# FibonacciDude/ContrastiveProsthetics

Measured on AMD Instinct MI355X. Metric: sEMG windows/sec contrastive step, 12-ch Ninapro, 1/2/4/8 MI355X, higher is better.
Workload: dtype bf16; 1 GPU; synthetic 12-ch sEMG, 41-class one-hot, batch 4096 groups/GPU (167936 windows/GPU/step), stock BN (--no_adabn), dp_emg=0.0635, d_e=16, random-init weights; global_batch_groups=4096, parallelism=dp1, loss=reference per-group loss, tile_schedule=static

## Files before the change

### contrastiveprosthetics_amd/csrc/conv_kernels.cuh

```cuda
#pragma once
#include <type_traits>
#include "common.cuh"
#include "gemm_tn.cuh"

#define CONV_WPB 16
#define CONV_ROWS (CONV_WPB * 12)
#define CONV_IMG_ROWS (CONV_WPB * 14)

struct ConvArgs {
    const float* x;
    const float* w1;
    const float* b1;
    const float* stats1;
    const void* wc;
    const float* bias2;
    const void* gin;
    const int* gin_exp;
    const float* coef;
    void* out;
    uint8_t* out8;
    const int* out_exp;
    uint32_t* out_amax;
    float* partials;
    int64_t n_windows;
// ... 449 lines not shown
    if constexpr (G8) gd = f8_exp2i(-*a.gin_exp);
    auto prefetch = [&](int64_t strip) {
        const int64_t win0 = strip * CONV_WG_WPB;
#pragma unroll
        for (int q = 0; q < NIT; ++q) {
            const int ir = rr + q * RPP;
            const int nl = ir / 14, wp = ir % 14;
            const int64_t win = win0 + nl;
            const bool ok = strip < nstrips && ir < CONV_WG_IMG && wp >= 1 && wp <= 12 && win < a.n_windows;
            const int64_t winc = ok ? win : 0;
            const int wpos = ok ? wp - 1 : 0;
            xg[q] = *(const GV*)((const unsigned char*)a.gin + ((winc * 12 + wpos) * 64 + cc * EPC) * (int64_t)sizeof(GV) / EPC);
            if constexpr (BN2) xr2[q] = *(const uint4*)((const T*)a.r2 + (winc * 12 + wpos) * 64 + cc * EPC);
            const float* xw = a.x + winc * 12;
            xr[q][0] = xw[wpos > 0 ? wpos - 1 : 0];
            xr[q][1] = xw[wpos];
            xr[q][2] = xw[wpos < 11 ? wpos + 1 : 11];
        }
    };
    prefetch(blockIdx.x);
    for (int64_t strip = blockIdx.x; strip < nstrips; strip += gridDim.x) {
        const int64_t win0 = strip * CONV_WG_WPB;
        {
#pragma unroll
            for (int q = 0; q < NIT; ++q) {
                const int ir = rr + q * RPP;
                const int nl = ir / 14, wp = ir % 14;
                const bool ok = ir < CONV_WG_IMG && wp >= 1 && wp <= 12 && win0 + nl < a.n_windows;
                const int wpos = ok ? wp - 1 : 0;
                float t[EPC];
                conv1_chunk_vals<T>(wpos > 0 ? xr[q][0] : 0.f, xr[q][1], wpos < 11 ? xr[q][2] : 0.f, wt, bs, t);
                if (a.stats1 != nullptr) {
#pragma unroll
                    for (int e = 0; e < EPC; ++e) t[e] = fmaf(t[e], sc[e], sh[e]);
                }
                uint4 yv = D::pack(t);
                uint4 xv;
                if constexpr (G8) xv = f8_chunk5_to_bf16(xg[q], gd);
                else xv = xg[q];
                if constexpr (BN2) {
                    float gv[EPC], rv[EPC];
                    D::unpack(xv, gv);
                    D::unpack(xr2[q], rv);
#pragma unroll
                    for (int e = 0; e < EPC; ++e) gv[e] = rv[e] > 0.f ? fmaf(c2a[e], gv[e], fmaf(c2b[e], rv[e], c2z[e])) : 0.f;
                    xv = D::pack(gv);
                    if (ok) {
                        *(uint4*)((T*)const_cast<void*>(a.gin) + ((win0 + nl) * 12 + wpos) * 64 + cc * EPC) = xv;
                        D::unpack(xv, gv);
#pragma unroll
                        for (int e = 0; e < EPC; ++e) {
                            cs_all[e] += gv[e];
                            cs_first[e] += wpos == 0 ? gv[e] : 0.f;
                            cs_last[e] += wpos == 11 ? gv[e] : 0.f;
                        }
                    }
                }
                if (!ok) { xv = make_uint4(0, 0, 0, 0); yv = make_uint4(0, 0, 0, 0); }
                if (ir < CONV_WG_IMG) {
                    *(uint4*)(Xi + (ir + 1) * PITCH + cc * 16) = xv;
                    *(uint4*)(Yi + (ir + 1) * PITCH + cc * 16) = yv;
                }
            }
        }
        __syncthreads();
        prefetch(strip + gridDim.x);
#pragma unroll
        for (int k0 = 0; k0 < CONV_WG_IMG; k0 += KSTEP) {
            uint4 fy;
            if constexpr (sizeof(T) == 2) fy = tn_frag_bf16<PITCH>(Yi, k0 + 1, it * 32, lane);
            else fy = tn_frag_f32<PITCH>(Yi, k0 + 1, it * 32, lane);
#pragma unroll
            for (int tap = 0; tap < 3; ++tap) {
                uint4 fx;
                if constexpr (sizeof(T) == 2) fx = tn_frag_bf16<PITCH>(Xi, k0 + 2 - tap, ot * 32, lane);
                else fx = tn_frag_f32<PITCH>(Xi, k0 + 2 - tap, ot * 32, lane);
                mma_chunk<T>(fx, fy, acc[tap]);
            }
        }
        __syncthreads();
    }
    float* slab = a.partials + (int64_t)blockIdx.x * 64 * 192;
    const int r = lane & 31, h = lane >> 5;
#pragma unroll
    for (int tap = 0; tap < 3; ++tap) {
        const int q = tap * 64 + it * 32 + r;
#pragma unroll
        for (int g = 0; g < 16; ++g) {
            const int p = ot * 32 + (g & 3) + 8 * (g >> 2) + 4 * h;
            slab[p * 192 + q] = acc[tap][g];
        }
    }
    if constexpr (BN2) {
        float* red = (float*)smem;
        static_assert(2 * ROWS * PITCH >= 3 * RPP * 64 * 4, "the column-sum reduction reuses the image region");
#pragma unroll
        for (int e = 0; e < EPC; ++e) {
            red[(0 * RPP + rr) * 64 + cc * EPC + e] = cs_all[e];
            red[(1 * RPP + rr) * 64 + cc * EPC + e] = cs_first[e];
            red[(2 * RPP + rr) * 64 + cc * EPC + e] = cs_last[e];
        }
        __syncthreads();
        if (tid < 192) {
            const int which = tid >> 6, c = tid & 63;
            float s = 0.f;
            for (int q = 0; q < RPP; ++q) s += red[(which * RPP + q) * 64 + c];
            a.gcols3[((int64_t)blockIdx.x * 3 + which) * 64 + c] = s;
        }
    }
}

template <typename T, bool G8 = false, bool ROWS = false>
__global__ __launch_bounds__(256, 2) void conv2_dgrad_conv1_kernel(ConvArgs a) {
    static_assert(!G8 || sizeof(T) == 2, "e5m2 gradients are expanded into a bf16 image");
    using GV = std::conditional_t<G8, uint2, uint4>;
    using D = DT<T>;
    using G = ConvGeo<T>;
    constexpr int EPC = G::EPC, CPR = G::CPR, ROWB = G::ROWB, RPP = G::RPP, WPITCH = G::WPITCH;
    constexpr int KSTEP = D::KSTEP, KS_PER_TAP = 64 / KSTEP, NKS = 3 * KS_PER_TAP;
    constexpr int IMG_BYTES = CONV_IMG_ROWS * ROWB, W_BYTES = 64 * WPITCH;
    __shared__ __attribute__((aligned(16))) unsigned char smem[IMG_BYTES + W_BYTES];
    __shared__ __attribute__((aligned(16))) float xpad[2][CONV_WPB * 16];
    static_assert(IMG_BYTES >= 4 * 8 * 32 * 4, "the end-of-kernel reduction reuses the image region");
    unsigned char* img = smem;
    unsigned char* Wl = smem + IMG_BYTES;
    float* red = (float*)smem;

    const int tid = threadIdx.x, lane = tid & 63, wave = tid >> 6;
    const int r = lane & 31, h = lane >> 5;
    const int cc = tid % CPR, rr = tid / CPR;
    const int ft = wave & 1, st0 = 3 * (wave >> 1);
    const int64_t nstrips = (a.n_windows + CONV_WPB - 1) / CONV_WPB;
    const int64_t total_rows = a.n_windows * 12;

    for (int i = tid; i < 64 * (192 / EPC); i += 256) {
        const int row = i / (192 / EPC), ch = i % (192 / EPC);
        *(uint4*)(Wl + row * WPITCH + ch * 16) = *(const uint4*)((const T*)a.wc + row * 192 + ch * EPC);
    }
    for (int i = tid; i < 2 * CONV_WPB * 16; i += 256) (&xpad[0][0])[i] = 0.f;
    const int ch1 = ft * 32 + r;
    const float w0 = a.w1[ch1 * 9 + 3], w1 = a.w1[ch1 * 9 + 4], w2 = a.w1[ch1 * 9 + 5], b1 = a.b1[ch1];
    float ca, cb, cz;
    if constexpr (ROWS) {
        __shared__ float ca_s[64], cb_s[64], cz_s[64];
        conv_bn_bwd_coef(a.rows1, a.rows1_nr, 1, a.stats1, (double)a.n_windows * 12, ca_s, cb_s, cz_s, (double (*)[4][64])smem, blockIdx.x == 0,
                         a.dgamma1, a.dbeta1);
        ca = ca_s[ch1]; cb = cb_s[ch1]; cz = cz_s[ch1];
        __syncthreads();
    } else {
        ca = a.coef[ch1]; cb = a.coef[64 + ch1]; cz = a.coef[128 + ch1];
    }
    float d0 = 0.f, d1 = 0.f, d2 = 0.f, d3 = 0.f;

    auto load_x = [&](int64_t strip) {
        const int64_t i = strip * (CONV_WPB * 12) + tid;
        return (tid < CONV_WPB * 12 && strip < nstrips && i < total_rows) ? a.x[i] : 0.f;
    };
    const int xslot = (tid / 12) * 16 + 1 + tid % 12;
    constexpr int NITG = CONV_IMG_ROWS / RPP;
    GV pg[NITG];
    float gd = 1.f;
    if constexpr (G8) gd = f8_exp2i(-*a.gin_exp);
    auto prefetch_g = [&](int64_t strip) {
#pragma unroll
        for (int it = 0; it < NITG; ++it) {
            const int ir = rr + it * RPP;
            const int nl = ir / 14, wp = ir % 14;
            const int64_t win = strip * CONV_WPB + nl;
            const bool ok = strip < nstrips && wp >= 1 && wp <= 12 && win < a.n_windows;
            pg[it] = *(const GV*)((const unsigned char*)a.gin + (((ok ? win : 0) * 12 + (ok ? wp - 1 : 0)) * 64 + cc * EPC) * (int64_t)sizeof(GV) / EPC);
            if (!ok) pg[it] = GV{};
        }
    };
    __syncthreads();
    if (tid < CONV_WPB * 12) xpad[0][xslot] = load_x(blockIdx.x);
    prefetch_g(blockIdx.x);
    int xb = 0;
    int ir0[3];
#pragma unroll
    for (int j = 0; j < 3; ++j) {
        const int ml = (st0 + j) * 32 + r;
        ir0[j] = (ml / 12) * 14 + (ml % 12);
    }
    for (int64_t strip = blockIdx.x; strip < nstrips; strip += gridDim.x) {
        const int64_t win0 = strip * CONV_WPB;
        const float x_next = load_x(strip + gridDim.x);
#pragma unroll
        for (int it = 0; it < NITG; ++it) {
            if constexpr (G8) *(uint4*)(img + G::img_off(rr + it * RPP, cc)) = f8_chunk5_to_bf16(pg[it], gd);
            else *(uint4*)(img + G::img_off(rr + it * RPP, cc)) = pg[it];
        }
        __syncthreads();
        prefetch_g(strip + gridDim.x);
        f32x16 acc[3];
#pragma unroll
        for (int j = 0; j < 3; ++j)
#pragma unroll
            for (int g = 0; g < 16; ++g) acc[j][g] = 0.f;
#pragma unroll
        for (int ks = 0; ks < NKS; ++ks) {
            const int tap = ks / KS_PER_TAP, chunk = (ks % KS_PER_TAP) * 2 + h;
            const uint4 fw = *(const uint4*)(Wl + (ft * 32 + r) * WPITCH + ks * 32 + h * 16);
#pragma unroll
            for (int j = 0; j < 3; ++j) {
                const uint4 fs = *(const uint4*)(img + G::img_off(ir0[j] + tap, chunk));
                mma_chunk<T>(fs, fw, acc[j]);
            }
        }
        if (tid < CONV_WPB * 12) xpad[xb ^ 1][xslot] = x_next;
        __syncthreads();
        const float* xs = xpad[xb];
#pragma unroll
        for (int j = 0; j < 3; ++j) {
#pragma unroll
            for (int q = 0; q < 4; ++q) {
                const int mb = (st0 + j) * 32 + 8 * q + 4 * h;
                const int nl = mb / 12, p0 = mb % 12;
                const bool valid = win0 + nl < a.n_windows;
                const float4 xa = *(const float4*)(xs + nl * 16 + p0);
                const float2 xc = *(const float2*)(xs + nl * 16 + p0 + 4);
                const float X[6] = {xa.x, xa.y, xa.z, xa.w, xc.x, xc.y};
#pragma unroll
                for (int e = 0; e < 4; e += 2) {
                    float y0 = fmaf(w2, X[e + 2], fmaf(w1, X[e + 1], fmaf(w0, X[e], b1)));
                    float y1 = fmaf(w2, X[e + 3], fmaf(w1, X[e + 2], fmaf(w0, X[e + 1], b1)));
                    float r0, r1;
                    if constexpr (sizeof(T) == 2) {
                        const uint32_t pk = cvt_pk_bf16<true>(y0, y1);
                        r0 = __uint_as_float(pk << 16);
                        r1 = __uint_as_float(pk & 0xffff0000u);
                    } else {
                        r0 = fmaxf(y0, 0.f);
                        r1 = fmaxf(y1, 0.f);
                    }
                    const float t0 = fmaf(ca, acc[j][4 * q + e], fmaf(cb, r0, cz));
                    const float t1 = fmaf(ca, acc[j][4 * q + e + 1], fmaf(cb, r1, cz));
                    const float g0 = (r0 > 0.f && valid) ? t0 : 0.f;
                    const float g1 = (r1 > 0.f && valid) ? t1 : 0.f;
                    d0 = fmaf(g0, X[e], d0);     d1 = fmaf(g0, X[e + 1], d1); d2 = fmaf(g0, X[e + 2], d2); d3 += g0;
                    d0 = fmaf(g1, X[e + 1], d0); d1 = fmaf(g1, X[e + 2], d1); d2 = fmaf(g1, X[e + 3], d2); d3 += g1;
                }
                __builtin_amdgcn_sched_barrier(0);
            }
        }
        xb ^= 1;
    }
    __syncthreads();
    red[(0 * 8 + wave * 2 + h) * 32 + r] = d0;
    red[(1 * 8 + wave * 2 + h) * 32 + r] = d1;
    red[(2 * 8 + wave * 2 + h) * 32 + r] = d2;
    red[(3 * 8 + wave * 2 + h) * 32 + r] = d3;
    __syncthreads();
    {
        const int k = tid >> 6, c = tid & 63, f = c >> 5, cl = c & 31;
        float s = 0.f;
#pragma unroll
        for (int wq = 0; wq < 2; ++wq)
#pragma unroll
            for (int hh = 0; hh < 2; ++hh) s += red[(k * 8 + (f + 2 * wq) * 2 + hh) * 32 + cl];
        a.partials[((int64_t)blockIdx.x * 4 + k) * 64 + c] = s;
    }
}
```

### contrastiveprosthetics_amd/csrc/gemm_nt.cuh

```cuda
#pragma once
#include "common.cuh"

enum { ALOAD_PLAIN = 0, ALOAD_CONV = 1,
       ALOAD_BNDROP = 2,
       ALOAD_F8 = 3,
       ALOAD_BNDROP_F8 = 4 };
enum { EPI_FWD = 0, EPI_DGRAD = 1, EPI_PLAIN_F32 = 2,
       EPI_DGRAD_BN = 3,
       EPI_DGRAD_ST = 4 };

struct GemmNTArgs {
    const void* A;
    const void* W;
    void* C;
    const float* bias;
    const void* R;
    float* partials;
    const float* coef;
    int coef_mod;
    const float* a_scale;
    const float* a_shift;
    const int* a_exp;
    int64_t M;
    int lda, ldc, ldr;
    int K, F;
    int relu;
    int f_valid;
    int pad0;
    uint32_t dp_thresh, dp_key;
    const uint32_t* dp_salt;
    float dp_inv_keep;
    int* sched;
};

template <typename T, int BM, int BN, int ALOAD, int EPI>
__global__ __launch_bounds__(256) void gemm_nt_kernel(GemmNTArgs a) {
    using D = DT<T>;
    constexpr int EPC = D::EPC;
    constexpr int BK = D::BK;
    constexpr int WAVES_F = (BN >= 128) ? 2 : 1;
    constexpr int WAVES_S = 4 / WAVES_F;
    constexpr int WS_T = BM / (WAVES_S * 32);
    constexpr int WF_T = BN / (WAVES_F * 32);
    constexpr int A_BYTES = BM * 128, W_BYTES = BN * 128;
    constexpr int C_PITCH = BN * (int)sizeof(T) + 16;
    constexpr int STAGE_BYTES = 2 * (A_BYTES + W_BYTES);
    constexpr int C_BYTES = (EPI == EPI_PLAIN_F32) ? 0 : BM * C_PITCH;
    constexpr int RED_BYTES = (EPI == EPI_PLAIN_F32) ? 0 : 2 * 256 * EPC * 4;
    constexpr int LDS_BYTES = (STAGE_BYTES > C_BYTES + RED_BYTES) ? STAGE_BYTES : (C_BYTES + RED_BYTES);
    static_assert(LDS_BYTES <= 160 * 1024, "LDS");
    __shared__ __attribute__((aligned(16))) unsigned char smem[LDS_BYTES];

    const int tid = threadIdx.x, lane = tid & 63, wave = tid >> 6;
    const int r = lane & 31, h = lane >> 5;
    const int tiles_f = a.F / BN;
    const int tile_f = blockIdx.x % tiles_f;
    const int64_t tile_m = blockIdx.x / tiles_f;
    const int64_t m0 = tile_m * BM;
    const int f0 = tile_f * BN;
    const int ws = wave / WAVES_F, wf = wave % WAVES_F;

    const T* __restrict__ Ag = (const T*)a.A;
    const T* __restrict__ Wg = (const T*)a.W;

    constexpr int A_IT = BM / 32, W_IT = BN / 32;
    uint4 areg[A_IT], wreg[W_IT];
    const int sc = tid & 7, sr = tid >> 3;
    float a_deq = 1.f;
    if constexpr (ALOAD == ALOAD_F8 || ALOAD == ALOAD_BNDROP_F8) a_deq = f8_exp2i(-*a.a_exp);

    auto load_tiles = [&](int kt) {
        const int k0 = kt * BK;
#pragma unroll
        for (int i = 0; i < W_IT; ++i) {
            const int row = sr + 32 * i;
            wreg[i] = *(const uint4*)(Wg + (int64_t)(f0 + row) * a.K + k0 + sc * EPC);
        }
#pragma unroll
        for (int i = 0; i < A_IT; ++i) {
            const int64_t m = m0 + sr + 32 * i;
            if constexpr (ALOAD == ALOAD_PLAIN || ALOAD == ALOAD_BNDROP || ALOAD == ALOAD_F8 || ALOAD == ALOAD_BNDROP_F8) {
                const int64_t mc = m < a.M ? m : a.M - 1;
                uint4 v;
                if constexpr (ALOAD == ALOAD_F8 || ALOAD == ALOAD_BNDROP_F8) {
                    static_assert(sizeof(T) == 2 || (ALOAD != ALOAD_F8 && ALOAD != ALOAD_BNDROP_F8), "e4m3 operands feed the bf16 kernels");
                    v = f8_chunk_to_bf16(*(const uint2*)((const uint8_t*)a.A + mc * a.lda + k0 + sc * 8), a_deq);
                } else {
                    v = *(const uint4*)(Ag + mc * a.lda + k0 + sc * EPC);
                }
                if constexpr (ALOAD == ALOAD_BNDROP || ALOAD == ALOAD_BNDROP_F8)
                    v = bn_drop_chunk<T>(v, a.a_scale, a.a_shift, k0 + sc * EPC, a.dp_salt ? (a.dp_key ^ *a.dp_salt) : a.dp_key, (uint32_t)mc,
                                         (uint32_t)a.K, a.dp_thresh, a.dp_inv_keep);
                if (m >= a.M) v = make_uint4(0, 0, 0, 0);
                areg[i] = v;
            } else {
                const int tap = k0 >> 6, ch0 = (k0 & 63) + sc * EPC;
                const int w = (int)(m % 12) + tap - 1;
                const bool ok = (m < a.M) && (w >= 0) && (w < 12);
                const int64_t ms = ok ? (m + tap - 1) : 0;
                uint4 v = *(const uint4*)(Ag + ms * a.lda + ch0);
                if (a.a_scale != nullptr) {
                    float x[EPC];
                    D::unpack(v, x);
#pragma unroll
                    for (int e = 0; e < EPC; ++e) x[e] = fmaf(x[e], a.a_scale[ch0 + e], a.a_shift[ch0 + e]);
                    v = D::pack(x);
                }
                if (!ok) v = make_uint4(0, 0, 0, 0);
                areg[i] = v;
            }
        }
    };
    auto store_tiles = [&](int buf) {
        unsigned char* As = smem + buf * (A_BYTES + W_BYTES);
        unsigned char* Ws = As + A_BYTES;
#pragma unroll
        for (int i = 0; i < A_IT; ++i) *(uint4*)(As + lds_tile_off(sr + 32 * i, sc)) = areg[i];
#pragma unroll
        for (int i = 0; i < W_IT; ++i) *(uint4*)(Ws + lds_tile_off(sr + 32 * i, sc)) = wreg[i];
    };

    f32x16 acc[WF_T][WS_T];
#pragma unroll
    for (int i = 0; i < WF_T; ++i)
#pragma unroll
        for (int j = 0; j < WS_T; ++j)
#pragma unroll
            for (int g = 0; g < 16; ++g) acc[i][j][g] = 0.f;

    const int nk = a.K / BK;
    load_tiles(0);
    store_tiles(0);
    __syncthreads();
    for (int kt = 0; kt < nk; ++kt) {
        if (kt + 1 < nk) load_tiles(kt + 1);
        const unsigned char* As = smem + (kt & 1) * (A_BYTES + W_BYTES);
        const unsigned char* Ws = As + A_BYTES;
#pragma unroll
        for (int ks = 0; ks < 4; ++ks) {
            uint4 fw[WF_T], fs[WS_T];
#pragma unroll
            for (int i = 0; i < WF_T; ++i)
                fw[i] = *(const uint4*)(Ws + lds_tile_off((wf * WF_T + i) * 32 + r, 2 * ks + h));
#pragma unroll
            for (int j = 0; j < WS_T; ++j)
                fs[j] = *(const uint4*)(As + lds_tile_off((ws * WS_T + j) * 32 + r, 2 * ks + h));
#pragma unroll
            for (int i = 0; i < WF_T; ++i)
#pragma unroll
                for (int j = 0; j < WS_T; ++j) mma_chunk<T>(fw[i], fs[j], acc[i][j]);
        }
        if (kt + 1 < nk) store_tiles((kt + 1) & 1);
        __syncthreads();
    }

    if constexpr (EPI == EPI_PLAIN_F32) {
        float* Cg = (float*)a.C;
#pragma unroll
        for (int i = 0; i < WF_T; ++i)
#pragma unroll
            for (int j = 0; j < WS_T; ++j) {
                const int64_t m = m0 + (ws * WS_T + j) * 32 + r;
#pragma unroll
                for (int q = 0; q < 4; ++q) {
                    const int f = f0 + (wf * WF_T + i) * 32 + 8 * q + 4 * h;
                    if (m < a.M && f < a.f_valid) {
                        float4 v = make_float4(acc[i][j][4 * q], acc[i][j][4 * q + 1], acc[i][j][4 * q + 2], acc[i][j][4 * q + 3]);
                        if (a.bias != nullptr) { v.x += a.bias[f]; v.y += a.bias[f + 1]; v.z += a.bias[f + 2]; v.w += a.bias[f + 3]; }
                        *(float4*)(Cg + m * a.ldc + f) = v;
                    }
                }
            }
        return;
    } else {
        unsigned char* Cs = smem;
        float* red = (float*)(smem + C_BYTES);
#pragma unroll
        for (int i = 0; i < WF_T; ++i)
#pragma unroll
            for (int j = 0; j < WS_T; ++j) {
                const int srow = (ws * WS_T + j) * 32 + r;
#pragma unroll
                for (int q = 0; q < 4; ++q) {
                    const int fl = (wf * WF_T + i) * 32 + 8 * q + 4 * h;
                    float v[4];
#pragma unroll
                    for (int e = 0; e < 4; ++e) {
                        float x = acc[i][j][4 * q + e];
                        if constexpr (EPI == EPI_FWD) {
                            x += a.bias[f0 + fl + e];
                            if (a.relu) x = fmaxf(x, 0.f);
                        }
                        v[e] = x;
                    }
                    unsigned char* dst = Cs + srow * C_PITCH + fl * (int)sizeof(T);
                    if constexpr (sizeof(T) == 2) {
                        *(uint2*)dst = make_uint2(pack2bf(v[0], v[1]), pack2bf(v[2], v[3]));
                    } else {
                        *(float4*)dst = make_float4(v[0], v[1], v[2], v[3]);
                    }
                }
            }
        __syncthreads();
        constexpr int CPR = BN / EPC;
        constexpr int RPP = 256 / CPR;
        const int cc = tid % CPR, rr = tid / CPR;
        float s1[EPC], s2[EPC];
#pragma unroll
        for (int e = 0; e < EPC; ++e) s1[e] = s2[e] = 0.f;
        T* Cg = (T*)a.C;
        const T* Rg = (const T*)a.R;
#pragma unroll 2
        for (int p = 0; p < BM / RPP; ++p) {
            const int row = rr + p * RPP;
            const int64_t m = m0 + row;
            if (m < a.M) {
                uint4 c = *(const uint4*)(Cs + row * C_PITCH + cc * 16);
                float v[EPC];
                D::unpack(c, v);
                const int f = f0 + cc * EPC;
                if constexpr (EPI == EPI_FWD) {
#pragma unroll
                    for (int e = 0; e < EPC; ++e) { s1[e] += v[e]; s2[e] = fmaf(v[e], v[e], s2[e]); }
                } else {
                    float rv[EPC];
                    uint4 rc = make_uint4(0, 0, 0, 0);
                    if (a.R != nullptr) rc = *(const uint4*)(Rg + m * a.ldr + f);
                    D::unpack(rc, rv);
                    if (a.dp_thresh != 0) {
#pragma unroll
                        for (int e = 0; e < EPC; e += 2) {
                            const uint32_t pr = dropout_pair(a.dp_salt ? (a.dp_key ^ *a.dp_salt) : a.dp_key, (uint32_t)m, (uint32_t)a.ldc, (uint32_t)(f + e));
                            v[e] *= dropout_scale(pr, 0, a.dp_thresh, a.dp_inv_keep);
                            v[e + 1] *= dropout_scale(pr, 1, a.dp_thresh, a.dp_inv_keep);
                        }
                        c = D::pack(v);
                    }
#pragma unroll
                    for (int e = 0; e < EPC; ++e) {
                        const float g = D::round(v[e]);
                        s1[e] += g;
                        s2[e] = fmaf(g, rv[e], s2[e]);
                    }
                }
                *(uint4*)(Cg + m * a.ldc + f) = c;
            }
        }
        if (EPI == EPI_DGRAD && a.R == nullptr) return;
#pragma unroll
        for (int e = 0; e < EPC; ++e) {
            red[(0 * RPP + rr) * BN + cc * EPC + e] = s1[e];
            red[(1 * RPP + rr) * BN + cc * EPC + e] = s2[e];
        }
        __syncthreads();
        if (tid < 2 * BN) {
            const int which = tid / BN, col = tid % BN;
            float s = 0.f;
#pragma unroll
            for (int q = 0; q < RPP; ++q) s += red[(which * RPP + q) * BN + col];
            a.partials[(tile_m * 2 + which) * a.F + f0 + col] = s;
        }
    }
}

template <typename T, int BM, int BN, int ALOAD, int EPI>
static inline hipError_t launch_gemm_nt(const GemmNTArgs& a, hipStream_t st) {
    const int64_t tiles_m = (a.M + BM - 1) / BM;
    const int64_t blocks = tiles_m * (a.F / BN);
    hipLaunchKernelGGL((gemm_nt_kernel<T, BM, BN, ALOAD, EPI>), dim3((unsigned)blocks), dim3(256), 0, st, a);
    return hipGetLastError();
}
```

### contrastiveprosthetics_amd/csrc/gemm_tn.cuh

```cuda
#pragma once
#include "common.cuh"

enum { YLOAD_PLAIN = 0, YLOAD_CONV = 1,
       YLOAD_BNDROP = 2,
       YLOAD_F8 = 3,
       YLOAD_BNDROP_F8 = 4 };

struct GemmTNArgs {
    const void* X;
    const void* Y;
    float* slabs;
    const float* y_scale;
    const float* y_shift;
    const int* y_exp;
    int64_t M;
    int64_t rows_per_split;
    int ldx, ldy, P, Q;
    uint32_t dp_thresh, dp_key;
    const uint32_t* dp_salt;
    float dp_inv_keep;
};

template <typename T, int COLS> struct TNPitch {
    static constexpr int value = (sizeof(T) == 2) ? COLS * 2 + 64 : COLS * 4 + 16;
// ... 39 lines not shown
    const int tp = blockIdx.x / tiles_q, tq = blockIdx.x % tiles_q;
    const int p0 = tp * BP, q0 = tq * BQ;
    const int64_t mb = (int64_t)blockIdx.y * a.rows_per_split;
    int64_t me = mb + a.rows_per_split;
    if (me > a.M) me = a.M;
    const int nsteps = (int)((me - mb + 31) / 32);

    const T* __restrict__ Xg = (const T*)a.X;
    const T* __restrict__ Yg = (const T*)a.Y;
    uint4 xreg[X_IT], yreg[Y_IT];
    float y_deq = 1.f;
    if constexpr (YLOAD == YLOAD_F8 || YLOAD == YLOAD_BNDROP_F8) y_deq = f8_exp2i(-*a.y_exp);

    auto load_tiles = [&](int step) {
        const int64_t ms = mb + (int64_t)step * 32;
#pragma unroll
        for (int i = 0; i < X_IT; ++i) {
            const int idx = tid + 256 * i;
            const int row = idx / XCPR, ch = idx % XCPR;
            const int64_t m = ms + row;
            uint4 v = make_uint4(0, 0, 0, 0);
            if (row < 32 && m < me) v = *(const uint4*)(Xg + m * a.ldx + p0 + ch * EPC);
            xreg[i] = v;
        }
#pragma unroll
        for (int i = 0; i < Y_IT; ++i) {
            const int idx = tid + 256 * i;
            const int row = idx / YCPR, ch = idx % YCPR;
            const int64_t m = ms + row;
            uint4 v = make_uint4(0, 0, 0, 0);
            if constexpr (YLOAD == YLOAD_PLAIN) {
                if (row < 32 && m < me) v = *(const uint4*)(Yg + m * a.ldy + q0 + ch * EPC);
            } else if constexpr (YLOAD == YLOAD_F8 || YLOAD == YLOAD_BNDROP_F8) {
                static_assert(sizeof(T) == 2 || (YLOAD != YLOAD_F8 && YLOAD != YLOAD_BNDROP_F8), "e4m3 operands feed the bf16 kernels");
                if (row < 32 && m < me) {
                    v = f8_chunk_to_bf16(*(const uint2*)((const uint8_t*)a.Y + m * a.ldy + q0 + ch * 8), y_deq);
                    if constexpr (YLOAD == YLOAD_BNDROP_F8)
                        v = bn_drop_chunk<T>(v, a.y_scale, a.y_shift, q0 + ch * EPC, a.dp_salt ? (a.dp_key ^ *a.dp_salt) : a.dp_key, (uint32_t)m,
                                             (uint32_t)a.Q, a.dp_thresh, a.dp_inv_keep);
                }
            } else if constexpr (YLOAD == YLOAD_BNDROP) {
                if (row < 32 && m < me)
                    v = bn_drop_chunk<T>(*(const uint4*)(Yg + m * a.ldy + q0 + ch * EPC), a.y_scale, a.y_shift, q0 + ch * EPC,
                                         a.dp_salt ? (a.dp_key ^ *a.dp_salt) : a.dp_key, (uint32_t)m, (uint32_t)a.Q, a.dp_thresh, a.dp_inv_keep);
            } else {
                const int tap = tq;
                const int w = (int)(m % 12) + tap - 1;
                if (row < 32 && m < me && w >= 0 && w < 12) {
                    v = *(const uint4*)(Yg + (m + tap - 1) * a.ldy + ch * EPC);
                    if (a.y_scale != nullptr) {
                        float x[EPC];
                        D::unpack(v, x);
#pragma unroll
                        for (int e = 0; e < EPC; ++e) x[e] = fmaf(x[e], a.y_scale[ch * EPC + e], a.y_shift[ch * EPC + e]);
                        v = D::pack(x);
                    }
                }
            }
            yreg[i] = v;
        }
    };
    auto store_tiles = [&](int buf) {
        unsigned char* Xs = smem + buf * (XB + YB);
        unsigned char* Ys = Xs + XB;
#pragma unroll
        for (int i = 0; i < X_IT; ++i) {
            const int idx = tid + 256 * i;
            const int row = idx / XCPR, ch = idx % XCPR;
            if (row < 32) *(uint4*)(Xs + row * PX + ch * 16) = xreg[i];
        }
#pragma unroll
        for (int i = 0; i < Y_IT; ++i) {
            const int idx = tid + 256 * i;
            const int row = idx / YCPR, ch = idx % YCPR;
            if (row < 32) *(uint4*)(Ys + row * PY + ch * 16) = yreg[i];
        }
    };

    f32x16 acc[WP_T][WQ_T];
#pragma unroll
    for (int i = 0; i < WP_T; ++i)
#pragma unroll
        for (int j = 0; j < WQ_T; ++j)
#pragma unroll
            for (int g = 0; g < 16; ++g) acc[i][j][g] = 0.f;

    if (nsteps > 0) {
        load_tiles(0);
        store_tiles(0);
    }
    __syncthreads();
    for (int step = 0; step < nsteps; ++step) {
        if (step + 1 < nsteps) load_tiles(step + 1);
        const unsigned char* Xs = smem + (step & 1) * (XB + YB);
        const unsigned char* Ys = Xs + XB;
#pragma unroll
        for (int ks = 0; ks < 32 / KSTEP; ++ks) {
            uint4 fx[WP_T], fy[WQ_T];
#pragma unroll
            for (int i = 0; i < WP_T; ++i) {
                const int c0 = (wp * WP_T + i) * 32;
                if constexpr (sizeof(T) == 2) fx[i] = tn_frag_bf16<PX>(Xs, ks * KSTEP, c0, lane);
                else fx[i] = tn_frag_f32<PX>(Xs, ks * KSTEP, c0, lane);
            }
#pragma unroll
            for (int j = 0; j < WQ_T; ++j) {
                const int c0 = (wq * WQ_T + j) * 32;
                if constexpr (sizeof(T) == 2) fy[j] = tn_frag_bf16<PY>(Ys, ks * KSTEP, c0, lane);
                else fy[j] = tn_frag_f32<PY>(Ys, ks * KSTEP, c0, lane);
            }
#pragma unroll
            for (int i = 0; i < WP_T; ++i)
#pragma unroll
                for (int j = 0; j < WQ_T; ++j) mma_chunk<T>(fx[i], fy[j], acc[i][j]);
        }
        if (step + 1 < nsteps) store_tiles((step + 1) & 1);
        __syncthreads();
    }

    float* slab = a.slabs + (int64_t)blockIdx.y * a.P * a.Q;
    const int r = lane & 31, h = lane >> 5;
#pragma unroll
    for (int i = 0; i < WP_T; ++i)
#pragma unroll
        for (int j = 0; j < WQ_T; ++j) {
            const int q = q0 + (wq * WQ_T + j) * 32 + r;
#pragma unroll
            for (int g = 0; g < 16; ++g) {
                const int p = p0 + (wp * WP_T + i) * 32 + (g & 3) + 8 * (g >> 2) + 4 * h;
                slab[(int64_t)p * a.Q + q] = acc[i][j][g];
            }
        }
}

template <typename T, int BP, int BQ, int YLOAD>
static inline hipError_t launch_gemm_tn(const GemmTNArgs& a, int splits, hipStream_t st) {
    dim3 grid((unsigned)((a.P / BP) * (a.Q / BQ)), (unsigned)splits);
    hipLaunchKernelGGL((gemm_tn_kernel<T, BP, BQ, YLOAD>), grid, dim3(256), 0, st, a);
    return hipGetLastError();
}

struct ProjWgradArgs {
    const bf16_t* dz;
    const void* R;
    float* slabs;
    int64_t M, rows_per_split;
    int splits;
    uint32_t dp_thresh, dp_key;
    const uint32_t* dp_salt;
};
#define PROJ_WGRAD_GRID(S) (32 * (((S) + 7) / 8))

template <bool F8>
__global__ __launch_bounds__(256) void proj_wgrad_sums_kernel(ProjWgradArgs a) {
    const int fx = (blockIdx.x >> 3) & 3, fy = (blockIdx.x >> 5) * 8 + (blockIdx.x & 7);
    if (fy >= a.splits) return;
    constexpr int PX = TNPitch<bf16_t, 32>::value, PY = TNPitch<bf16_t, 128>::value;
    constexpr int XB = 32 * PX, YB = 32 * PY, BUF = XB + 2 * YB;
    __shared__ __attribute__((aligned(16))) unsigned char smem[2 * BUF];
    const int tid = threadIdx.x, lane = tid & 63, wave = tid >> 6;
    const int q0 = fx * 128;
    const int64_t mb = (int64_t)fy * a.rows_per_split;
    int64_t me = mb + a.rows_per_split;
    if (me > a.M) me = a.M;
    const int nsteps = (int)((me - mb + 31) / 32);
    const uint32_t key = a.dp_salt ? (a.dp_key ^ *a.dp_salt) : a.dp_key;
    uint4 xreg, ya[2], yb[2];
    auto load_tiles = [&](int step) {
        const int64_t ms = mb + (int64_t)step * 32;
        {
            const int row = tid >> 2, ch = tid & 3;
            const int64_t m = ms + row;
            xreg = make_uint4(0, 0, 0, 0);
            if (tid < 128 && m < me) xreg = *(const uint4*)(a.dz + m * 64 + ch * 8);
        }
#pragma unroll
        for (int i = 0; i < 2; ++i) {
            const int idx = tid + 256 * i, row = idx >> 4, ch = idx & 15;
            const int64_t m = ms + row;
            uint4 v = make_uint4(0, 0, 0, 0), o = make_uint4(0, 0, 0, 0);
            if (m < me) {
                if constexpr (F8) v = f8_chunk_to_bf16(*(const uint2*)((const uint8_t*)a.R + m * 512 + q0 + ch * 8), 1.f);
                else v = *(const uint4*)((const bf16_t*)a.R + m * 512 + q0 + ch * 8);
                const uint2 d0 = dropout_quad(key, (uint32_t)m, 512u, (uint32_t)(q0 + ch * 8));
                const uint2 d1 = dropout_quad(key, (uint32_t)m, 512u, (uint32_t)(q0 + ch * 8 + 4));
                auto word_mask = [&](uint32_t dr) {
                    return ((dr & 0xFFFFu) >= a.dp_thresh ? 0xFFFFu : 0u) | ((dr >> 16) >= a.dp_thresh ? 0xFFFF0000u : 0u);
                };
                const uint32_t m0 = word_mask(d0.x), m1 = word_mask(d0.y), m2 = word_mask(d1.x), m3 = word_mask(d1.y);
                v = make_uint4(v.x & m0, v.y & m1, v.z & m2, v.w & m3);
                o = make_uint4(0x3F803F80u & m0, 0x3F803F80u & m1, 0x3F803F80u & m2, 0x3F803F80u & m3);
            }
            ya[i] = v;
            yb[i] = o;
        }
    };
    auto store_tiles = [&](int buf) {
        unsigned char* Xs = smem + buf * BUF;
        unsigned char* As = Xs + XB;
        unsigned char* Bs = As + YB;
        if (tid < 128) *(uint4*)(Xs + (tid >> 2) * PX + (tid & 3) * 16) = xreg;
#pragma unroll
        for (int i = 0; i < 2; ++i) {
            const int idx = tid + 256 * i, row = idx >> 4, ch = idx & 15;
            *(uint4*)(As + row * PY + ch * 16) = ya[i];
            *(uint4*)(Bs + row * PY + ch * 16) = yb[i];
        }
    };
    f32x16 accA, accB;
#pragma unroll
    for (int g = 0; g < 16; ++g) accA[g] = accB[g] = 0.f;
    if (nsteps > 0) {
        load_tiles(0);
        store_tiles(0);
    }
    __syncthreads();
    for (int step = 0; step < nsteps; ++step) {
        if (step + 1 < nsteps) load_tiles(step + 1);
        const unsigned char* Xs = smem + (step & 1) * BUF;
        const unsigned char* As = Xs + XB;
        const unsigned char* Bs = As + YB;
#pragma unroll
        for (int ks = 0; ks < 2; ++ks) {
            const uint4 fx = tn_frag_bf16<PX>(Xs, ks * 16, 0, lane);
            const uint4 fa = tn_frag_bf16<PY>(As, ks * 16, wave * 32, lane);
            const uint4 fb = tn_frag_bf16<PY>(Bs, ks * 16, wave * 32, lane);
            mma_chunk<bf16_t>(fx, fa, accA);
            mma_chunk<bf16_t>(fx, fb, accB);
        }
        if (step + 1 < nsteps) store_tiles((step + 1) & 1);
        __syncthreads();
    }
    float* slab = a.slabs + (int64_t)fy * 32 * 512;
    const int r = lane & 31, h = lane >> 5, q = q0 + wave * 32 + r;
#pragma unroll
    for (int g = 0; g < 8; ++g) {
        const int pcol = (g & 3) + 8 * (g >> 2) + 4 * h;
        slab[pcol * 512 + q] = accA[g];
        slab[(16 + pcol) * 512 + q] = accB[g];
    }
}

#define PROJ_FINISH_ROWS 4
__global__ __launch_bounds__(256) void proj_wgrad_finish_kernel(const float* __restrict__ slabs, int S, const float* __restrict__ scale,
                                                                const float* __restrict__ shift, const float* __restrict__ Wp,
                                                                float inv_keep, const int* __restrict__ r_exp, float* __restrict__ dWp,
                                                                float* __restrict__ rows) {
    __shared__ float part[2][4][4][16];
    __shared__ float red[2][4][16];
    const int tid = threadIdx.x, fl = tid & 15, jl = (tid >> 4) & 3, sh = tid >> 6;
    const int f = blockIdx.x * 16 + fl, j = blockIdx.y * 4 + jl;
    const float* pa = slabs + j * 512 + f;
    const float* pb = pa + 16 * 512;
    const int64_t sstride = 32 * 512;
    float a0 = 0.f, a1 = 0.f, b0 = 0.f, b1 = 0.f;
    int k = sh;
    for (; k + 28 < S; k += 32) {
        float va[8], vb[8];
#pragma unroll
        for (int u = 0; u < 8; ++u) { va[u] = pa[(k + 4 * u) * sstride]; vb[u] = pb[(k + 4 * u) * sstride]; }
        a0 += (va[0] + va[2]) + (va[4] + va[6]);
        a1 += (va[1] + va[3]) + (va[5] + va[7]);
        b0 += (vb[0] + vb[2]) + (vb[4] + vb[6]);
        b1 += (vb[1] + vb[3]) + (vb[5] + vb[7]);
    }
    for (; k < S; k += 4) { a0 += pa[k * sstride]; b0 += pb[k * sstride]; }
    part[0][sh][jl][fl] = a0 + a1;
    part[1][sh][jl][fl] = b0 + b1;
    __syncthreads();
    if (sh == 0) {
        const float A = ((part[0][0][jl][fl] + part[0][1][jl][fl]) + (part[0][2][jl][fl] + part[0][3][jl][fl])) * inv_keep * (r_exp ? f8_exp2i(-*r_exp) : 1.f);
        const float B = ((part[1][0][jl][fl] + part[1][1][jl][fl]) + (part[1][2][jl][fl] + part[1][3][jl][fl])) * inv_keep;
        dWp[j * 512 + f] = fmaf(scale[f], A, shift[f] * B);
        const float w = bf2f(f2bf(Wp[j * 512 + f]));
        red[0][jl][fl] = w * B;
        red[1][jl][fl] = w * A;
    }
    __syncthreads();
    if (tid < 32) {
        const int which = tid >> 4, c = tid & 15;
        rows[((int64_t)blockIdx.y * 2 + which) * 512 + blockIdx.x * 16 + c] = (red[which][0][c] + red[which][1][c]) + (red[which][2][c] + red[which][3][c]);
    }
}
```

Before: 48.59 million windows/s.

## Deepen load pipelines and defer BN/dropout transform until the LDS store

In the NT GEMM's BN+dropout A-load path, raw operands are now loaded early and the scale/shift/dropout is applied at store time, after the MMA loop, behind a scheduling barrier. This keeps the transform arithmetic off the global-load issue path. The projection wgrad sums kernel gets a two-stage register prefetch (loads two steps ahead) with deferred fp8 decode and masking, plus an occupancy hint of 3 blocks per CU. The conv kernel precomputes gather offsets and uses clamped, always-valid addresses with masking applied at store, removing per-load branches. The price is higher register pressure, which may limit occupancy or cause spills.

```diff
diff --git a/contrastiveprosthetics_amd/csrc/conv_kernels.cuh b/contrastiveprosthetics_amd/csrc/conv_kernels.cuh
--- a/contrastiveprosthetics_amd/csrc/conv_kernels.cuh
+++ b/contrastiveprosthetics_amd/csrc/conv_kernels.cuh
@@ -625,28 +625,33 @@
     }
     float d0 = 0.f, d1 = 0.f, d2 = 0.f, d3 = 0.f;
 
-    auto load_x = [&](int64_t strip) {
-        const int64_t i = strip * (CONV_WPB * 12) + tid;
-        return (tid < CONV_WPB * 12 && strip < nstrips && i < total_rows) ? a.x[i] : 0.f;
-    };
+    auto x_live = [&](int64_t strip) { return tid < CONV_WPB * 12 && strip < nstrips && strip * (CONV_WPB * 12) + tid < total_rows; };
+    auto load_x = [&](int64_t strip) { return a.x[x_live(strip) ? strip * (CONV_WPB * 12) + tid : 0]; };
     const int xslot = (tid / 12) * 16 + 1 + tid % 12;
     constexpr int NITG = CONV_IMG_ROWS / RPP;
     GV pg[NITG];
     float gd = 1.f;
     if constexpr (G8) gd = f8_exp2i(-*a.gin_exp);
+    constexpr int GVB = (int)sizeof(GV);
+    uint32_t goff[NITG], wp_live = 0;
+#pragma unroll
+    for (int it = 0; it < NITG; ++it) {
+        const int ir = rr + it * RPP;
+        const int nl = ir / 14, wp = ir % 14;
+        const int pos = wp < 1 ? 0 : (wp > 12 ? 11 : wp - 1);
+        goff[it] = (uint32_t)(((nl * 12 + pos) * 64 + cc * EPC) * GVB / EPC);
+        wp_live |= (wp >= 1 && wp <= 12) ? (1u << it) : 0u;
+    }
     auto prefetch_g = [&](int64_t strip) {
-#pragma unroll
-        for (int it = 0; it < NITG; ++it) {
-            const int ir = rr + it * RPP;
-            const int nl = ir / 14, wp = ir % 14;
-            const int64_t win = strip * CONV_WPB + nl;
-            const bool ok = strip < nstrips && wp >= 1 && wp <= 12 && win < a.n_windows;
-            pg[it] = *(const GV*)((const unsigned char*)a.gin + (((ok ? win : 0) * 12 + (ok ? wp - 1 : 0)) * 64 + cc * EPC) * (int64_t)sizeof(GV) / EPC);
-            if (!ok) pg[it] = GV{};
-        }
+        const int64_t sc = strip < nstrips ? strip : 0;
+        const int64_t left = a.n_windows - sc * CONV_WPB;
+        const uint32_t last = (uint32_t)(left < CONV_WPB ? left : CONV_WPB) * (12 * 64 * GVB / EPC) - GVB;
+        const unsigned char* base = (const unsigned char*)a.gin + sc * (CONV_WPB * 12 * 64 * GVB / EPC);
+#pragma unroll
+        for (int it = 0; it < NITG; ++it) pg[it] = *(const GV*)(base + (goff[it] < last ? goff[it] : last));
     };
     __syncthreads();
-    if (tid < CONV_WPB * 12) xpad[0][xslot] = load_x(blockIdx.x);
+    if (tid < CONV_WPB * 12) xpad[0][xslot] = x_live(blockIdx.x) ? load_x(blockIdx.x) : 0.f;
     prefetch_g(blockIdx.x);
     int xb = 0;
     int ir0[3];
@@ -658,10 +663,14 @@
     for (int64_t strip = blockIdx.x; strip < nstrips; strip += gridDim.x) {
         const int64_t win0 = strip * CONV_WPB;
         const float x_next = load_x(strip + gridDim.x);
+        const int live_rows = (int)(a.n_windows - win0 < CONV_WPB ? a.n_windows - win0 : CONV_WPB) * 14;
 #pragma unroll
         for (int it = 0; it < NITG; ++it) {
-            if constexpr (G8) *(uint4*)(img + G::img_off(rr + it * RPP, cc)) = f8_chunk5_to_bf16(pg[it], gd);
-            else *(uint4*)(img + G::img_off(rr + it * RPP, cc)) = pg[it];
+            const int ir = rr + it * RPP;
+            const bool ok = ((wp_live >> it) & 1u) && rr < live_rows - it * RPP;
+            const GV v = ok ? pg[it] : GV{};
+            if constexpr (G8) *(uint4*)(img + G::img_off(ir, cc)) = f8_chunk5_to_bf16(v, gd);
+            else *(uint4*)(img + G::img_off(ir, cc)) = v;
         }
         __syncthreads();
         prefetch_g(strip + gridDim.x);
@@ -680,7 +689,7 @@
                 mma_chunk<T>(fs, fw, acc[j]);
             }
         }
-        if (tid < CONV_WPB * 12) xpad[xb ^ 1][xslot] = x_next;
+        if (tid < CONV_WPB * 12) xpad[xb ^ 1][xslot] = x_live(strip + gridDim.x) ? x_next : 0.f;
         __syncthreads();
         const float* xs = xpad[xb];
 #pragma unroll
diff --git a/contrastiveprosthetics_amd/csrc/gemm_nt.cuh b/contrastiveprosthetics_amd/csrc/gemm_nt.cuh
--- a/contrastiveprosthetics_amd/csrc/gemm_nt.cuh
+++ b/contrastiveprosthetics_amd/csrc/gemm_nt.cuh
@@ -69,30 +69,52 @@
     float a_deq = 1.f;
     if constexpr (ALOAD == ALOAD_F8 || ALOAD == ALOAD_BNDROP_F8) a_deq = f8_exp2i(-*a.a_exp);
 
+    constexpr bool LATE_A = ALOAD == ALOAD_BNDROP || ALOAD == ALOAD_BNDROP_F8;
+    f32x2_t a_sc[LATE_A ? EPC / 2 : 1], a_sh[LATE_A ? EPC / 2 : 1], a_keep[LATE_A ? A_IT : 1][LATE_A ? EPC / 2 : 1];
     auto load_tiles = [&](int kt) {
         const int k0 = kt * BK;
 #pragma unroll
         for (int i = 0; i < W_IT; ++i) {
             const int row = sr + 32 * i;
             wreg[i] = *(const uint4*)(Wg + (int64_t)(f0 + row) * a.K + k0 + sc * EPC);
+        }
+        if constexpr (LATE_A) {
+            const int f = k0 + sc * EPC;
+            const uint32_t key = a.dp_salt ? (a.dp_key ^ *a.dp_salt) : a.dp_key;
+#pragma unroll
+            for (int e = 0; e < EPC; e += 2) {
+                a_sc[e / 2] = (f32x2_t){a.a_scale[f + e], a.a_scale[f + e + 1]};
+                a_sh[e / 2] = (f32x2_t){a.a_shift[f + e], a.a_shift[f + e + 1]};
+            }
+#pragma unroll
+            for (int i = 0; i < A_IT; ++i) {
+                const int64_t m = m0 + sr + 32 * i;
+                const int64_t mc = m < a.M ? m : a.M - 1;
+#pragma unroll
+                for (int e = 0; e < EPC; e += 2) {
+                    const uint32_t pr = dropout_pair(key, (uint32_t)mc, (uint32_t)a.K, (uint32_t)(f + e));
+                    a_keep[i][e / 2] = (f32x2_t){dropout_scale(pr, 0, a.dp_thresh, a.dp_inv_keep), dropout_scale(pr, 1, a.dp_thresh, a.dp_inv_keep)};
+                }
+            }
         }
 #pragma unroll
         for (int i = 0; i < A_IT; ++i) {
             const int64_t m = m0 + sr + 32 * i;
             if constexpr (ALOAD == ALOAD_PLAIN || ALOAD == ALOAD_BNDROP || ALOAD == ALOAD_F8 || ALOAD == ALOAD_BNDROP_F8) {
                 const int64_t mc = m < a.M ? m : a.M - 1;
-                uint4 v;
-                if constexpr (ALOAD == ALOAD_F8 || ALOAD == ALOAD_BNDROP_F8) {
-                    static_assert(sizeof(T) == 2 || (ALOAD != ALOAD_F8 && ALOAD != ALOAD_BNDROP_F8), "e4m3 operands feed the bf16 kernels");
-                    v = f8_chunk_to_bf16(*(const uint2*)((const uint8_t*)a.A + mc * a.lda + k0 + sc * 8), a_deq);
+                static_assert(sizeof(T) == 2 || (ALOAD != ALOAD_F8 && ALOAD != ALOAD_BNDROP_F8), "e4m3 operands feed the bf16 kernels");
+                if constexpr (ALOAD == ALOAD_BNDROP_F8) {
+                    const uint2 raw = *(const uint2*)((const uint8_t*)a.A + mc * a.lda + k0 + sc * 8);
+                    areg[i] = make_uint4(raw.x, raw.y, 0, 0);
+                } else if constexpr (ALOAD == ALOAD_BNDROP) {
+                    areg[i] = *(const uint4*)(Ag + mc * a.lda + k0 + sc * EPC);
                 } else {
-                    v = *(const uint4*)(Ag + mc * a.lda + k0 + sc * EPC);
-                }
-                if constexpr (ALOAD == ALOAD_BNDROP || ALOAD == ALOAD_BNDROP_F8)
-                    v = bn_drop_chunk<T>(v, a.a_scale, a.a_shift, k0 + sc * EPC, a.dp_salt ? (a.dp_key ^ *a.dp_salt) : a.dp_key, (uint32_t)mc,
-                                         (uint32_t)a.K, a.dp_thresh, a.dp_inv_keep);
-                if (m >= a.M) v = make_uint4(0, 0, 0, 0);
-                areg[i] = v;
+                    uint4 v;
+                    if constexpr (ALOAD == ALOAD_F8) v = f8_chunk_to_bf16(*(const uint2*)((const uint8_t*)a.A + mc * a.lda + k0 + sc * 8), a_deq);
+                    else v = *(const uint4*)(Ag + mc * a.lda + k0 + sc * EPC);
+                    if (m >= a.M) v = make_uint4(0, 0, 0, 0);
+                    areg[i] = v;
+                }
             } else {
                 const int tap = k0 >> 6, ch0 = (k0 & 63) + sc * EPC;
                 const int w = (int)(m % 12) + tap - 1;
@@ -111,9 +133,28 @@
             }
         }
     };
-    auto store_tiles = [&](int buf) {
-        unsigned char* As = smem + buf * (A_BYTES + W_BYTES);
+    auto store_tiles = [&](int kt) {
+        unsigned char* As = smem + (kt & 1) * (A_BYTES + W_BYTES);
         unsigned char* Ws = As + A_BYTES;
+        if constexpr (LATE_A) {
+#pragma unroll
+            for (int i = 0; i < A_IT; ++i) {
+                const int64_t m = m0 + sr + 32 * i;
+                uint4 v = areg[i];
+                if constexpr (ALOAD == ALOAD_BNDROP_F8) v = f8_chunk_to_bf16(make_uint2(v.x, v.y), a_deq);
+                float x[EPC];
+                D::unpack(v, x);
+#pragma unroll
+                for (int e = 0; e < EPC; e += 2) {
+                    const f32x2_t y = __builtin_elementwise_fma((f32x2_t){x[e], x[e + 1]}, a_sc[e / 2], a_sh[e / 2]) * a_keep[i][e / 2];
+                    x[e] = y.x;
+                    x[e + 1] = y.y;
+                }
+                v = D::pack(x);
+                if (m >= a.M) v = make_uint4(0, 0, 0, 0);
+                areg[i] = v;
+            }
+        }
 #pragma unroll
         for (int i = 0; i < A_IT; ++i) *(uint4*)(As + lds_tile_off(sr + 32 * i, sc)) = areg[i];
 #pragma unroll
@@ -150,7 +191,8 @@
 #pragma unroll
                 for (int j = 0; j < WS_T; ++j) mma_chunk<T>(fw[i], fs[j], acc[i][j]);
         }
-        if (kt + 1 < nk) store_tiles((kt + 1) & 1);
+        if constexpr (LATE_A) __builtin_amdgcn_sched_barrier(0);
+        if (kt + 1 < nk) store_tiles(kt + 1);
         __syncthreads();
     }
 
diff --git a/contrastiveprosthetics_amd/csrc/gemm_tn.cuh b/contrastiveprosthetics_amd/csrc/gemm_tn.cuh
--- a/contrastiveprosthetics_amd/csrc/gemm_tn.cuh
+++ b/contrastiveprosthetics_amd/csrc/gemm_tn.cuh
@@ -215,7 +215,7 @@
 #define PROJ_WGRAD_GRID(S) (32 * (((S) + 7) / 8))
 
 template <bool F8>
-__global__ __launch_bounds__(256) void proj_wgrad_sums_kernel(ProjWgradArgs a) {
+__global__ __launch_bounds__(256, 3) void proj_wgrad_sums_kernel(ProjWgradArgs a) {
     const int fx = (blockIdx.x >> 3) & 3, fy = (blockIdx.x >> 5) * 8 + (blockIdx.x & 7);
     if (fy >= a.splits) return;
     constexpr int PX = TNPitch<bf16_t, 32>::value, PY = TNPitch<bf16_t, 128>::value;
@@ -228,58 +228,64 @@
     if (me > a.M) me = a.M;
     const int nsteps = (int)((me - mb + 31) / 32);
     const uint32_t key = a.dp_salt ? (a.dp_key ^ *a.dp_salt) : a.dp_key;
-    uint4 xreg, ya[2], yb[2];
-    auto load_tiles = [&](int step) {
+    using YV = std::conditional_t<F8, uint2, uint4>;
+    struct Stage {
+        uint4 x;
+        YV y[2];
+        uint32_t mk[2][4];
+    };
+    Stage sa, sb;
+    auto load_tiles = [&](int step, Stage& s) {
         const int64_t ms = mb + (int64_t)step * 32;
         {
-            const int row = tid >> 2, ch = tid & 3;
-            const int64_t m = ms + row;
-            xreg = make_uint4(0, 0, 0, 0);
-            if (tid < 128 && m < me) xreg = *(const uint4*)(a.dz + m * 64 + ch * 8);
+            const int row = (tid & 127) >> 2, ch = tid & 3;
+            const int64_t m = ms + row < me ? ms + row : me - 1;
+            s.x = *(const uint4*)(a.dz + m * 64 + ch * 8);
+        }
+#pragma unroll
+        for (int i = 0; i < 2; ++i) {
+            const int idx = tid + 256 * i, row = idx >> 4, ch = idx & 15;
+            const int64_t m = ms + row < me ? ms + row : me - 1;
+            if constexpr (F8) s.y[i] = *(const uint2*)((const uint8_t*)a.R + m * 512 + q0 + ch * 8);
+            else s.y[i] = *(const uint4*)((const bf16_t*)a.R + m * 512 + q0 + ch * 8);
         }
 #pragma unroll
         for (int i = 0; i < 2; ++i) {
             const int idx = tid + 256 * i, row = idx >> 4, ch = idx & 15;
             const int64_t m = ms + row;
-            uint4 v = make_uint4(0, 0, 0, 0), o = make_uint4(0, 0, 0, 0);
-            if (m < me) {
-                if constexpr (F8) v = f8_chunk_to_bf16(*(const uint2*)((const uint8_t*)a.R + m * 512 + q0 + ch * 8), 1.f);
-                else v = *(const uint4*)((const bf16_t*)a.R + m * 512 + q0 + ch * 8);
-                const uint2 d0 = dropout_quad(key, (uint32_t)m, 512u, (uint32_t)(q0 + ch * 8));
-                const uint2 d1 = dropout_quad(key, (uint32_t)m, 512u, (uint32_t)(q0 + ch * 8 + 4));
-                auto word_mask = [&](uint32_t dr) {
-                    return ((dr & 0xFFFFu) >= a.dp_thresh ? 0xFFFFu : 0u) | ((dr >> 16) >= a.dp_thresh ? 0xFFFF0000u : 0u);
-                };
-                const uint32_t m0 = word_mask(d0.x), m1 = word_mask(d0.y), m2 = word_mask(d1.x), m3 = word_mask(d1.y);
-                v = make_uint4(v.x & m0, v.y & m1, v.z & m2, v.w & m3);
-                o = make_uint4(0x3F803F80u & m0, 0x3F803F80u & m1, 0x3F803F80u & m2, 0x3F803F80u & m3);
-            }
-            ya[i] = v;
-            yb[i] = o;
-        }
-    };
-    auto store_tiles = [&](int buf) {
-        unsigned char* Xs = smem + buf * BUF;
+            const uint32_t live = m < me ? 0xFFFFFFFFu : 0u;
+            const uint2 d0 = dropout_quad(key, (uint32_t)m, 512u, (uint32_t)(q0 + ch * 8));
+            const uint2 d1 = dropout_quad(key, (uint32_t)m, 512u, (uint32_t)(q0 + ch * 8 + 4));
+            auto word_mask = [&](uint32_t dr) {
+                return (((dr & 0xFFFFu) >= a.dp_thresh ? 0xFFFFu : 0u) | ((dr >> 16) >= a.dp_thresh ? 0xFFFF0000u : 0u)) & live;
+            };
+            s.mk[i][0] = word_mask(d0.x); s.mk[i][1] = word_mask(d0.y); s.mk[i][2] = word_mask(d1.x); s.mk[i][3] = word_mask(d1.y);
+        }
+    };
+    auto store_tiles = [&](int step, const Stage& s) {
+        unsigned char* Xs = smem + (step & 1) * BUF;
         unsigned char* As = Xs + XB;
         unsigned char* Bs = As + YB;
-        if (tid < 128) *(uint4*)(Xs + (tid >> 2) * PX + (tid & 3) * 16) = xreg;
+        if (tid < 128) {
+            const bool live = mb + (int64_t)step * 32 + (tid >> 2) < me;
+            *(uint4*)(Xs + (tid >> 2) * PX + (tid & 3) * 16) = live ? s.x : make_uint4(0, 0, 0, 0);
+        }
 #pragma unroll
         for (int i = 0; i < 2; ++i) {
             const int idx = tid + 256 * i, row = idx >> 4, ch = idx & 15;
-            *(uint4*)(As + row * PY + ch * 16) = ya[i];
-            *(uint4*)(Bs + row * PY + ch * 16) = yb[i];
+            uint4 v;
+            if constexpr (F8) v = f8_chunk_to_bf16(s.y[i], 1.f);
+            else v = s.y[i];
+            const uint32_t m0 = s.mk[i][0], m1 = s.mk[i][1], m2 = s.mk[i][2], m3 = s.mk[i][3];
+            *(uint4*)(As + row * PY + ch * 16) = make_uint4(v.x & m0, v.y & m1, v.z & m2, v.w & m3);
+            *(uint4*)(Bs + row * PY + ch * 16) = make_uint4(0x3F803F80u & m0, 0x3F803F80u & m1, 0x3F803F80u & m2, 0x3F803F80u & m3);
         }
     };
     f32x16 accA, accB;
 #pragma unroll
     for (int g = 0; g < 16; ++g) accA[g] = accB[g] = 0.f;
-    if (nsteps > 0) {
-        load_tiles(0);
-        store_tiles(0);
-    }
-    __syncthreads();
-    for (int step = 0; step < nsteps; ++step) {
-        if (step + 1 < nsteps) load_tiles(step + 1);
+    auto do_step = [&](int step, Stage& nxt, const Stage& cur) {
+        load_tiles(step + 2, nxt);
         const unsigned char* Xs = smem + (step & 1) * BUF;
         const unsigned char* As = Xs + XB;
         const unsigned char* Bs = As + YB;
@@ -291,8 +297,19 @@
             mma_chunk<bf16_t>(fx, fa, accA);
             mma_chunk<bf16_t>(fx, fb, accB);
         }
-        if (step + 1 < nsteps) store_tiles((step + 1) & 1);
+        __builtin_amdgcn_sched_barrier(0);
+        store_tiles(step + 1, cur);
         __syncthreads();
+    };
+    load_tiles(0, sa);
+    load_tiles(1, sb);
+    store_tiles(0, sa);
+    __syncthreads();
+    for (int step = 0;;) {
+        if (step >= nsteps) break;
+        do_step(step++, sa, sb);
+        if (step >= nsteps) break;
+        do_step(step++, sb, sa);
     }
     float* slab = a.slabs + (int64_t)fy * 32 * 512;
     const int r = lane & 31, h = lane >> 5, q = q0 + wave * 32 + r;
```

Result: no change. 48.79 million windows/s (median of 6 runs) (+0.4%).
